# Sirui-Xu/InterDiff

Measured on AMD Instinct MI355X. Metric: denoising frame-steps/sec (denoising-steps/sec x B x T frames), higher is better.
Workload: dtype f32 (every contraction of the denoiser -- feed-forward block, QKV projection, self-attention, row-block contractions and the two token GEMMs: every fp32 operand as two f16 planes, 3 f16 MFMAs per product, fp32 accumulate; SMPL and everything else fp32 MFMA / VALU)

## Files before the change

### include/interdiff_hip.h

```cpp
#ifndef INTERDIFF_HIP_H
#define INTERDIFF_HIP_H

#include <stddef.h>
#include <stdint.h>

#ifdef __cplusplus
extern "C" {
#endif

#define IDF_OK            0
#define IDF_E_INVAL      -22
#define IDF_E_NOMEM      -12
#define IDF_E_LAUNCH     -5

int         interdiff_abi_version(void);
const char *interdiff_build_info(void);

int interdiff_rotation_6d_to_matrix   (const float *d6, float *m,  int64_t n, void *stream);
int interdiff_matrix_to_rotation_6d   (const float *m,  float *d6, int64_t n, void *stream);
int interdiff_matrix_to_axis_angle    (const float *m,  float *aa, int64_t n, void *stream);
int interdiff_axis_angle_to_matrix    (const float *aa, float *m,  int64_t n, void *stream);
int interdiff_axis_angle_to_quaternion(const float *aa, float *q,  int64_t n, void *stream);
int interdiff_rotation_6d_to_axis_angle(const float *d6, float *aa, int64_t n, void *stream);

typedef struct {
    int32_t V, J, n_betas, KB, S;
    const float   *blend;
    const float   *jt;
    const float   *js;
    const int32_t *parents;
    const int32_t *skin_idx;
    const float   *skin_w;
} idf_smpl_model;

size_t interdiff_smpl_workspace_bytes(const idf_smpl_model *m, int64_t N);
int interdiff_smpl_forward(const idf_smpl_model *m, const float *pose, const float *betas,
                           const float *trans, int64_t N, float *verts, float *jtr,
                           float *v_posed, void *ws, size_t ws_bytes, void *stream);

int interdiff_vertex_normals(const float *verts, int64_t N, int32_t V, const int32_t *faces,
                             const int32_t *adj_ptr, const int32_t *adj_face,
                             const int32_t *adj_corner, float *normals, void *stream);
int interdiff_nn_argmin(const float *q, int32_t Pq, const float *r, int32_t Pr, int64_t N,
                        int32_t *idx, void *stream);
int interdiff_point2point_signed(const float *x, int32_t P1, const float *y, int32_t P2, int64_t N,
                                 const float *x_normals, const float *y_normals,
                                 float *y2x_signed, float *x2y_signed, int32_t *yidx, int32_t *xidx,
                                 float *y2x, float *x2y, void *stream);

#define IDF_MDM_LAYERS 8
#define IDF_MDM_D      256
#define IDF_MDM_FF     1024
#define IDF_MDM_HEADS  4
#define IDF_MDM_NQ     10
#define IDF_MDM_MEM    10
#define IDF_MDM_MEM_MAX 16
#define IDF_FFN_SLICES 5

typedef struct {
    int64_t is_qan;
    int64_t sa_in_w, sa_in_b, sa_out_w, sa_out_b;
    int64_t qc, wk;
    int64_t ca_q_w, ca_q_b;
    int64_t ca_kv_w, ca_kv_b;
    int64_t ca_out_w, ca_out_b;
    int64_t ff1_w, ff1_b, ff2_w, ff2_b;
    int64_t ffn_pack;
    int64_t ffn_b1p;
    int64_t sa_in_pack;
    int64_t sa_out_frag;
    int64_t ln_w[3], ln_b[3];
    int64_t ffn_pack_h2;
    int64_t sa_in_pack_h2;
    int64_t qc_h2;
    int64_t rb_h2_ok;
    int64_t sa_out_frag_h2;
    int64_t qkv_bounds_ok;
} idf_mdm_layer;

typedef struct {
    int32_t C;
    int32_t n_steps;
    const float *arena;
    int64_t in_w, in_b;
    int64_t out_w, out_b;
// ... 188 lines not shown
```

### interdiff_amd/_lib.py

```python
import ctypes as C
import os
import torch

_HERE = os.path.dirname(os.path.abspath(__file__))
LIB_PATH = os.environ.get('INTERDIFF_HIP_LIB') or os.path.join(_HERE, 'csrc', 'libinterdiff_hip.so')
ABI_VERSION = 16

vp, i32, i64, f32, u64, sz = C.c_void_p, C.c_int32, C.c_int64, C.c_float, C.c_uint64, C.c_size_t

MDM_LAYERS = 8
FFN_SLICES = 5
STEP_EMBED_READY, STEP_EMBED_NEXT = 1, 2
TUNE = dict(embed=0, qkv=1, outproj=2, ffn=3, ffn_math=4, heads=5, contact=6, misc=7)


class SmplModel(C.Structure):
    _fields_ = [('V', i32), ('J', i32), ('n_betas', i32), ('KB', i32), ('S', i32),
                ('blend', vp), ('jt', vp), ('js', vp), ('parents', vp), ('skin_idx', vp), ('skin_w', vp)]


class MdmLayer(C.Structure):
    _fields_ = [('is_qan', i64),
                ('sa_in_w', i64), ('sa_in_b', i64), ('sa_out_w', i64), ('sa_out_b', i64),
                ('qc', i64), ('wk', i64),
                ('ca_q_w', i64), ('ca_q_b', i64), ('ca_kv_w', i64), ('ca_kv_b', i64),
                ('ca_out_w', i64), ('ca_out_b', i64),
                ('ff1_w', i64), ('ff1_b', i64), ('ff2_w', i64), ('ff2_b', i64), ('ffn_pack', i64), ('ffn_b1p', i64), ('sa_in_pack', i64), ('sa_out_frag', i64),
                ('ln_w', i64 * 3), ('ln_b', i64 * 3), ('ffn_pack_h2', i64), ('sa_in_pack_h2', i64), ('qc_h2', i64), ('rb_h2_ok', i64), ('sa_out_frag_h2', i64), ('qkv_bounds_ok', i64)]


class MdmWeights(C.Structure):
    _fields_ = [('C', i32), ('n_steps', i32), ('arena', vp),
                ('in_w', i64), ('in_b', i64), ('out_w', i64), ('out_b', i64),
                ('temb_table', i64), ('pe', i64), ('max_T', i32), ('has_encoder', i32),
                ('layer', MdmLayer * MDM_LAYERS), ('enc_layer', MdmLayer * MDM_LAYERS), ('tune', i32 * 8), ('out_w_h2', i64), ('in_w_h2', i64), ('tail_h2_ok', i64), ('mem_len', i32), ('rb_tokens', i32)]


class PnMlp(C.Structure):
    _fields_ = [('w', i64 * 3), ('b', i64 * 3), ('c', i32 * 4)]


class PointNet2(C.Structure):
    _fields_ = [('arena', vp), ('sa1', PnMlp * 2), ('sa2', PnMlp * 2), ('lin_w', i64), ('lin_b', i64)]


class ObjProj(C.Structure):
    _fields_ = [('T', i32), ('past_len', i32), ('P', i32), ('n_pre', i32), ('arena', vp),
                ('dct_pad', i64), ('dct', i64), ('idct', i64), ('hand_bonus', i64),
                ('layer', i64 * 12), ('cin', i32 * 12), ('cout', i32 * 12)]


class CorrectionCtx(C.Structure):
    _fields_ = [('smpl', C.POINTER(SmplModel)), ('objproj', C.POINTER(ObjProj)),
                ('faces', vp), ('adj_ptr', vp), ('adj_face', vp), ('adj_corner', vp), ('markers_idx', vp),
                ('n_markers', i32), ('n_points', i32), ('past_len', i32), ('tune', i32),
                ('vorder', vp), ('faces_scan', vp), ('markers_scan', vp), ('adj_pair_scan', vp), ('adj_pair', vp), ('vrank', vp)]


class OptCtx(C.Structure):
    _fields_ = [('geo', C.POINTER(CorrectionCtx)), ('blendT', vp), ('jv_ptr', vp), ('jv_vtx', vp), ('jv_w', vp), ('K3P', i32), ('_pad', i32)]


OPT_NP, OPT_NLOSS = 483, 6
_OPT_PTRS = ('betas', 'obj_points', 'param', 'init', 'grad', 'm', 'v', 'best', 'pose', 'tr', 'verts', 'vposed', 'verts_gt', 'gv',
             'jtr', 'pts', 'y2x', 'y2x_signed', 'yidx', 'near', 'dvposed', 'dA', 'dfeat', 'gtr', 'lossf', 'loss', 'loss_hist',
             'best_loss', 'flag', 'foot_static', 'foot_cnt', 'ctl', 'smpl_ws')


class OptState(C.Structure):
    _fields_ = [('B', i32), ('T', i32), ('P', i32), ('max_iters', i32)] + [(k, vp) for k in _OPT_PTRS] + [('smpl_ws_bytes', sz), ('porder', vp), ('psort', vp), ('pbox', vp)]

# ... 128 lines not shown
```

### interdiff_amd/csrc/denoiser.hip

```cpp
#include "common.h"
#include "gemm.h"
#include "ffn.h"
#include "ffn_h2.h"
#include "tail_h2.h"
#include "attn_h2.h"

static inline int idf_launch_layer_ffn(hipStream_t s, const idf_mdm_layer &ly, const float *ar, const int32_t *tune, const float *x2, int M, float *parts) {
    int rows = idf_ffn::ffn_rows_of_tune(tune[IDF_TUNE_FFN]);
    if (tune[IDF_TUNE_FFN_MATH] != 0 && ly.ffn_pack_h2 != 0) {
        const int rc = idf_ffn_h2::launch_ffn_h2(s, x2, M, ar + ly.ffn_pack_h2, ar + ly.ffn_b1p, ar + ly.ff2_b, parts, rows ? rows : idf_ffn::ffn_tile_for_rows(M), tune[IDF_TUNE_MISC] == 2 ? 1 : (tune[IDF_TUNE_MISC] == 3 ? 2 : (tune[IDF_TUNE_MISC] == 6 ? 3 : (tune[IDF_TUNE_MISC] == 10 ? 4 : 0))));
        if (rc != IDF_NOT_EXCLUSIVE) return rc;
    }
    idf_ffn::launch_ffn(s, x2, M, ar + ly.ffn_pack, ar + ly.ffn_b1p, ar + ly.ff2_b, parts, rows);
    return IDF_OK;
}
#include <float.h>
#ifndef IDF_LDS_STRIDE_SET
#define IDF_LDS_STRIDE_SET 5
#endif

#ifndef IDF_AT_STAMP
#define IDF_AT_STAMP(i) do { } while (0)
#endif
#ifndef IDF_RB_STAMP
// ... 1793 lines not shown
            run_heads_post(tune[IDF_TUNE_GEMM_HEADS], s, g, u_np);
        } else {
            run_gemm_ln<E_HEADS>(pick(tune[IDF_TUNE_GEMM_HEADS], CFG_HEADS), s, g, u_np);
        }
    }
    idf_prof_mark(-1, s);
    IDF_CHECK_LAUNCH();
    return IDF_OK;
}
int mdm_forward_impl(const idf_mdm_weights *w, const float *memctx, const float *x, const int64_t *ts, int32_t B, int32_t T, float *x0,
                     void *ws, size_t ws_bytes, void *stream, const StepPost &post, int32_t flags = 0) {
    if (!w || w->mem_len < 0 || w->mem_len > MEMX) return IDF_E_INVAL;
    return idf_mem_len(w) == MEM ? mdm_forward_impl_t<MEM>(w, memctx, x, ts, B, T, x0, ws, ws_bytes, stream, post, flags)
                                 : mdm_forward_impl_t<MEMX>(w, memctx, x, ts, B, T, x0, ws, ws_bytes, stream, post, flags);
}
}

extern "C" int interdiff_mdm_forward(const idf_mdm_weights *w, const float *memctx, const float *x, const int64_t *ts,
                                     int32_t B, int32_t T, float *x0, void *ws, size_t ws_bytes, void *stream) {
    if (!x0) return IDF_E_INVAL;
    return mdm_forward_impl(w, memctx, x, ts, B, T, x0, ws, ws_bytes, stream, StepPost{});
}

extern "C" int interdiff_mdm_forward_step(const idf_mdm_weights *w, const float *memctx, float *x, int64_t *ts, int32_t B, int32_t T,
                                          const float *gt, const uint8_t *mask, const float *table, int64_t *state, void *ws,
                                          size_t ws_bytes, void *stream) {
    if (!x || !ts || !table || !state || (mask && !gt) || T <= 0) return IDF_E_INVAL;
    if (!(T & 3) && ((reinterpret_cast<uintptr_t>(x) | reinterpret_cast<uintptr_t>(gt)) & 15 || (reinterpret_cast<uintptr_t>(mask) & 3))) return IDF_E_INVAL;
    if ((reinterpret_cast<uintptr_t>(x) | reinterpret_cast<uintptr_t>(gt)) & 3) return IDF_E_INVAL;
    if (!w || w->layer[0].is_qan) return IDF_E_INVAL;
    return mdm_forward_impl(w, memctx, x, ts, B, T, nullptr, ws, ws_bytes, stream, StepPost{x, gt, mask, table, state, ts});
}

extern "C" int interdiff_mdm_forward_step_ex(const idf_mdm_weights *w, const float *memctx, float *x, int64_t *ts, int32_t B, int32_t T,
                                             const float *gt, const uint8_t *mask, const float *table, int64_t *state, void *ws,
                                             size_t ws_bytes, int32_t flags, void *stream) {
    if (!x || !ts || !table || !state || (mask && !gt) || T <= 0 || (flags & ~(IDF_STEP_EMBED_READY | IDF_STEP_EMBED_NEXT))) return IDF_E_INVAL;
    if (!(T & 3) && ((reinterpret_cast<uintptr_t>(x) | reinterpret_cast<uintptr_t>(gt)) & 15 || (reinterpret_cast<uintptr_t>(mask) & 3))) return IDF_E_INVAL;
    if ((reinterpret_cast<uintptr_t>(x) | reinterpret_cast<uintptr_t>(gt)) & 3) return IDF_E_INVAL;
    if (!w || w->layer[0].is_qan) return IDF_E_INVAL;
    return mdm_forward_impl(w, memctx, x, ts, B, T, nullptr, ws, ws_bytes, stream, StepPost{x, gt, mask, table, state, ts}, flags);
}

extern "C" int interdiff_mdm_step_chaining(const idf_mdm_weights *w) {
    return w && w->tune[IDF_TUNE_FFN_MATH] != 0 && w->out_w_h2 != 0 && w->in_w_h2 != 0 && w->C == idf_tail_h2::CW && w->tail_h2_ok != 0 &&
                   idf_tail_h2::tail_exclusive_ok(false) && idf_tail_h2::tail_exclusive_ok(true) ? 1 : 0;
}

extern "C" int interdiff_debug_deny_exclusive(const char *patterns) {
    idf_excl_set_deny(patterns);
    return IDF_OK;
}

extern "C" int interdiff_exclusive_cu_report(char *buf, int32_t cap) {
    if (!buf || cap <= 0) return IDF_E_INVAL;
    {
        static idf_excl_cache c[7];
        using namespace idf_ffn_h2;
        idf_exclusive_cu(reinterpret_cast<const void *>(&ffn_h2_kernel<1, FFN_H2_SLOTS, 0>), "ffn_h2_kernel<16 rows>", NT, c[0]);
        idf_exclusive_cu(reinterpret_cast<const void *>(&ffn_h2_kernel<2, FFN_H2_SLOTS, 0>), "ffn_h2_kernel<32 rows>", NT, c[1]);
        idf_exclusive_cu(reinterpret_cast<const void *>(&ffn_h2_kernel<2, FFN_H2_SLOTS, 0, 8>), "ffn_h2_kernel<32 rows, loader waves>", NT + 512, c[6]);
        idf_exclusive_cu(reinterpret_cast<const void *>(&ffn_h2_kernel<4, 2, 0>), "ffn_h2_kernel<64 rows>", NT, c[2]);
        idf_exclusive_cu(reinterpret_cast<const void *>(&ln_linear_h2_kernel<1, false, IDF_QKV_LOADER_WAVES>), "ln_linear_h2_kernel<1 slab>", NT + 64 * IDF_QKV_LOADER_WAVES, c[3]);
        idf_exclusive_cu(reinterpret_cast<const void *>(&ln_linear_h2_kernel<IDF_FFN_SLICES, false, IDF_QKV_LOADER_WAVES>), "ln_linear_h2_kernel<5 slabs>", NT + 64 * IDF_QKV_LOADER_WAVES, c[4]);
        idf_exclusive_cu(reinterpret_cast<const void *>(&idf_attn_h2::self_attn_h2_kernel<0, false>), "self_attn_h2_kernel", idf_attn_h2::NTH, c[5]);
    }
    qkv_planes_ok(1, 1, 16);
    qkv_planes_ok(NSL, 1, 16);
    rb_h2_qan_dyn<MEM>();
    rb_h2_std_dyn<MEM>();
    rb_h2_qan_dyn<MEMX>();
    rb_h2_std_dyn<MEMX>();
    rb8_qan_dyn<MEM, 16>();
    rb8_std_dyn<MEM, 16>();
    rb8_qan_dyn<MEM, 8>();
    rb8_std_dyn<MEM, 8>();
    rb8_qan_dyn<MEMX, 16>();
    rb8_std_dyn<MEMX, 16>();
    rb8_qan_dyn<MEMX, 8>();
    rb8_std_dyn<MEMX, 8>();
    idf_tail_h2::tail_exclusive_ok(false);
    idf_tail_h2::tail_exclusive_ok(true);
    return idf_excl_report(buf, cap);
}
```

### interdiff_amd/csrc/optimize.hip

```cpp
#include "common.h"
#include "rot_math.h"
#include "rot_dual.h"
#include <cfloat>

namespace {

constexpr int NP = IDF_OPT_NP, NL = IDF_OPT_NLOSS, NJ = 52, MAXJ = 64;
constexpr int OFF_TR = 468, OFF_OT = 471, OFF_OR = 474;
constexpr int FOOT0 = 10;
constexpr int KSLICE = 1024;

__device__ __forceinline__ float sgn(float x) { return x > 0.f ? 1.f : (x < 0.f ? -1.f : 0.f); }

__global__ __launch_bounds__(64) void opt_init_kernel(const float *__restrict__ pose, const float *__restrict__ trans,
                                                      const float *__restrict__ obj_angles, const float *__restrict__ obj_trans,
                                                      float *__restrict__ param, float *__restrict__ init, float *__restrict__ best) {
    const int64_t n = blockIdx.x;
    const int j = threadIdx.x;
    float out[9];
    int off = -1, cnt = 0;
    if (j < NJ || j == NJ + 2) {
        const float *a = j < NJ ? pose + n * 156 + 3 * j : obj_angles + n * 3;
        float q[4];
        rot::axis_angle_to_quaternion(a, q);
// ... 536 lines not shown
            float *h = loss_hist + ((size_t)it * B + b) * 4;
            h[0] = total; h[1] = col; h[2] = reg; h[3] = regv;
        }
        if (flag) {
            const int better = ctl[0] > 150 && total < best_loss[b];
            if (better) best_loss[b] = total;
            flag[b] = better;
        }
    }
}

__global__ __launch_bounds__(256) void opt_save_kernel(const float *__restrict__ param, float *__restrict__ best, const int32_t *__restrict__ flag,
                                                       int T, int64_t total, int32_t *__restrict__ ctl) {
    const int64_t i = (int64_t)blockIdx.x * 256 + threadIdx.x;
    if (i < total && flag[(i / NP) / T]) best[i] = param[i];
    if (i == 0) { ctl[0] += 1; ctl[1] += 1; }
}

__global__ __launch_bounds__(64) void opt_finish_kernel(const float *__restrict__ best, float *__restrict__ pose, float *__restrict__ trans,
                                                        float *__restrict__ obj_angles, float *__restrict__ obj_trans) {
    const int64_t n = blockIdx.x;
    const int j = threadIdx.x;
    const float *p = best + n * NP;
    if (j < NJ) rot::matrix_to_axis_angle(p + 9 * j, pose + n * 156 + 3 * j);
    else if (j == NJ) rot::matrix_to_axis_angle(p + OFF_OR, obj_angles + n * 3);
    else if (j < NJ + 4) {
        const int c = j - NJ - 1;
        trans[n * 3 + c] = p[OFF_TR + c];
        obj_trans[n * 3 + c] = p[OFF_OT + c];
    }
}

bool valid(const idf_opt_ctx *c, const idf_opt_state *st) {
    if (!c || !st || !c->geo || !c->geo->smpl || !c->blendT || !c->jv_ptr || !c->jv_vtx || !c->jv_w) return false;
    const idf_smpl_model *m = c->geo->smpl;
    if (m->J != NJ || m->n_betas != 10 || m->KB % 16 != 0 || c->K3P % KSLICE != 0 || c->K3P < 3 * m->V) return false;
    if (st->B < 1 || st->T < 3 || st->P < 1 || (size_t)m->V * 3 * sizeof(float) > 150 * 1024) return false;
    const void *need[] = {st->betas, st->obj_points, st->param, st->init, st->grad, st->m, st->v, st->best, st->pose, st->tr, st->verts,
                          st->vposed, st->verts_gt, st->gv, st->jtr, st->pts, st->y2x, st->y2x_signed, st->near,
                          st->yidx, st->dvposed, st->dA, st->dfeat, st->gtr, st->lossf, st->loss, st->best_loss, st->flag,
                          st->foot_static, st->foot_cnt, st->ctl, st->smpl_ws};
    for (const void *p : need)
        if (!p) return false;
    return st->smpl_ws_bytes >= interdiff_smpl_workspace_bytes(m, (int64_t)st->B * st->T);
}

int loss_grad(const idf_opt_ctx *c, const idf_opt_state *st, void *stream, bool bookkeeping) {
    const idf_smpl_model *m = c->geo->smpl;
    const int64_t N = (int64_t)st->B * st->T;
    const int V = m->V, J = m->J, P = st->P, T = st->T;
    hipStream_t s = idf_stream(stream);
    hipLaunchKernelGGL(opt_unpack_kernel, dim3((unsigned)N), dim3(64), 0, s, st->param, st->pose, st->tr);
    hipLaunchKernelGGL(opt_objpts_kernel, dim3((unsigned)idf_cdiv(P, 256), (unsigned)N), dim3(256), 0, s, st->param, st->obj_points, P, T, st->pts);
    int rc = interdiff_smpl_forward(m, st->pose, st->betas, st->tr, N, st->verts, st->jtr, st->vposed, st->smpl_ws, st->smpl_ws_bytes, stream);
    if (rc) return rc;
    if (c->geo->vorder && st->porder && st->psort && st->pbox) {
        rc = idf_nn_scan_opt(s, N, T, st->verts, V, st->pts, st->obj_points, P, st->porder, c->geo, st->yidx);
        if (rc) return rc;
        rc = idf_near_mask_opt(s, N, T, st->verts, V, st->pts, P, st->porder, c->geo->vorder, st->psort, st->pbox, st->near);
        if (rc) return rc;
    } else {
        if (hipMemsetAsync(st->near, 0, (size_t)N * V * sizeof(int32_t), s) != hipSuccess) return IDF_E_LAUNCH;
        hipLaunchKernelGGL(opt_nn_kernel, dim3((unsigned)idf_cdiv(P, NN_T * 2), (unsigned)N), dim3(NN_T), 0, s, st->pts, P, st->verts, V, st->yidx,
                           st->near);
    }
    hipLaunchKernelGGL(opt_signed_kernel, dim3((unsigned)idf_cdiv(P, 256), (unsigned)N), dim3(256), 0, s, st->pts, P, st->verts, V, st->yidx,
                       c->geo->faces, c->geo->adj_ptr, c->geo->adj_face, c->geo->adj_corner, c->geo->adj_pair, st->y2x_signed, st->y2x);
    static std::atomic<uint64_t> lds_ok{0};
    if (idf_opt_in_lds(reinterpret_cast<const void *>(opt_lossgrad_kernel), 150 * 1024, lds_ok) != IDF_OK) return IDF_E_LAUNCH;
    hipLaunchKernelGGL(opt_lossgrad_kernel, dim3((unsigned)N), dim3(LG_T), (size_t)V * 3 * sizeof(float), s, st->verts, st->verts_gt, V,
                       st->y2x_signed, st->near, st->yidx, st->y2x, st->obj_points, P, T, st->ctl, st->gv, st->grad, st->gtr, st->lossf);
    const float *A = reinterpret_cast<const float *>(reinterpret_cast<const char *>(st->smpl_ws) + idf_align((size_t)N * m->KB * sizeof(float)));
    hipLaunchKernelGGL(opt_skin_vertex_kernel, dim3((unsigned)idf_cdiv(V, 256), (unsigned)N), dim3(256), 0, s, *m, A, st->gv, c->K3P, st->dvposed);
    hipLaunchKernelGGL(opt_skin_joint_kernel, dim3((unsigned)J, (unsigned)N), dim3(64), 0, s, c->jv_ptr, c->jv_vtx, c->jv_w, st->gv, st->vposed, V,
                       J, st->dA);
    const int n_slices = c->K3P / KSLICE;
    hipLaunchKernelGGL(opt_dfeat_kernel, dim3((unsigned)(m->KB / 16), (unsigned)n_slices, (unsigned)idf_cdiv(N, 16 * DF_MT)), dim3(256), 0, s,
                       st->dvposed, c->blendT, (int)N, m->KB, c->K3P, st->dfeat);
    hipLaunchKernelGGL(opt_chain_bwd_kernel, dim3((unsigned)N), dim3(64), 0, s, *m, st->pose, st->betas, st->param, st->dA, st->dfeat, n_slices, N,
                       T, st->jtr, st->foot_static, st->foot_cnt, st->gtr, st->grad, st->lossf);
    hipLaunchKernelGGL(opt_reg_kernel, dim3((unsigned)N), dim3(512), 0, s, st->param, st->init, T, st->grad, st->lossf);
    hipLaunchKernelGGL(opt_loss_kernel, dim3((unsigned)st->B), dim3(64), 0, s, st->lossf, T, st->B, st->ctl, st->max_iters, st->loss,
                       bookkeeping ? st->loss_hist : nullptr, st->best_loss, bookkeeping ? st->flag : nullptr);
    IDF_CHECK_LAUNCH();
    return IDF_OK;
}

}

extern "C" int interdiff_optimize_init(const idf_opt_ctx *c, const idf_opt_state *st, const float *pose, const float *trans,
                                       const float *obj_angles, const float *obj_trans, int32_t first_iter, void *stream) {
    if (!valid(c, st) || !pose || !trans || !obj_angles || !obj_trans) return IDF_E_INVAL;
    const idf_smpl_model *m = c->geo->smpl;
    const int64_t N = (int64_t)st->B * st->T;
    hipStream_t s = idf_stream(stream);
    hipLaunchKernelGGL(opt_init_kernel, dim3((unsigned)N), dim3(64), 0, s, pose, trans, obj_angles, obj_trans, st->param, st->init, st->best);
    const size_t pb = (size_t)N * NP * sizeof(float);
    if (hipMemsetAsync(st->m, 0, pb, s) != hipSuccess || hipMemsetAsync(st->v, 0, pb, s) != hipSuccess ||
        hipMemsetAsync(st->grad, 0, pb, s) != hipSuccess ||
        hipMemsetAsync(st->dvposed, 0, (size_t)N * c->K3P * sizeof(float), s) != hipSuccess ||
        hipMemsetAsync(st->flag, 0, (size_t)st->B * sizeof(int32_t), s) != hipSuccess)
        return IDF_E_LAUNCH;
    hipLaunchKernelGGL(opt_setctl_kernel, dim3(1), dim3(64), 0, s, st->ctl, first_iter);
    if (c->geo->vorder && st->porder && idf_point_order(s, st->obj_points, st->B, st->P, st->porder) != IDF_OK) return IDF_E_INVAL;
    const int rc = interdiff_smpl_forward(m, pose, st->betas, trans, N, st->verts_gt, st->jtr, nullptr, st->smpl_ws, st->smpl_ws_bytes, stream);
    if (rc) return rc;
    hipLaunchKernelGGL(opt_static_kernel, dim3((unsigned)st->B), dim3(64), 0, s, st->jtr, st->T, m->J, st->foot_static, st->foot_cnt,
                       st->best_loss);
    IDF_CHECK_LAUNCH();
    return IDF_OK;
}

extern "C" int interdiff_optimize_loss_grad(const idf_opt_ctx *c, const idf_opt_state *st, void *stream) {
    if (!valid(c, st)) return IDF_E_INVAL;
    return loss_grad(c, st, stream, false);
}

extern "C" int interdiff_optimize_step(const idf_opt_ctx *c, const idf_opt_state *st, void *stream) {
    if (!valid(c, st)) return IDF_E_INVAL;
    const int rc = loss_grad(c, st, stream, true);
    if (rc) return rc;
    const int64_t total = (int64_t)st->B * st->T * NP;
    hipStream_t s = idf_stream(stream);
    hipLaunchKernelGGL(opt_adam_kernel, dim3((unsigned)idf_cdiv(total, 256)), dim3(256), 0, s, st->param, st->grad, st->m, st->v, total, st->ctl);
    hipLaunchKernelGGL(opt_save_kernel, dim3((unsigned)idf_cdiv(total, 256)), dim3(256), 0, s, st->param, st->best, st->flag, st->T, total, st->ctl);
    IDF_CHECK_LAUNCH();
    return IDF_OK;
}

extern "C" int interdiff_optimize_finish(const idf_opt_ctx *c, const idf_opt_state *st, float *pose, float *trans, float *obj_angles,
                                         float *obj_trans, void *stream) {
    if (!valid(c, st) || !pose || !trans || !obj_angles || !obj_trans) return IDF_E_INVAL;
    hipLaunchKernelGGL(opt_finish_kernel, dim3((unsigned)((int64_t)st->B * st->T)), dim3(64), 0, idf_stream(stream), st->best, pose, trans,
                       obj_angles, obj_trans);
    IDF_CHECK_LAUNCH();
    return IDF_OK;
}

extern "C" int interdiff_debug_joint_map_vjp(const float *R, const float *g_out, float *g_in, int32_t n) {
    if (!R || !g_out || !g_in || n < 0) return IDF_E_INVAL;
    for (int i = 0; i < n; ++i) rotd::joint_map_vjp(R + 9 * i, g_out + 9 * i, g_in + 9 * i);
    return IDF_OK;
}
```

### interdiff_amd/csrc/smpl.hip

```cpp
#include "common.h"
#include "rot_math.h"
#include <algorithm>

#ifndef IDF_SMPL_STAMP
#define IDF_SMPL_STAMP(i) do { } while (0)
#endif

namespace {

constexpr int MAXJ = 64;

__global__ __launch_bounds__(64) void smpl_pose_kernel(const idf_smpl_model m, const float *__restrict__ pose,
                                                       const float *__restrict__ betas, const float *__restrict__ trans,
                                                       float *__restrict__ feat, float *__restrict__ A,
                                                       float *__restrict__ jtr) {
    __shared__ float Rs[MAXJ * 9], Js[MAXJ * 3], Gs[MAXJ * 12];
    const int64_t n = blockIdx.x;
    const int j = threadIdx.x, J = m.J, nb = m.n_betas, KB = m.KB;
    const float *beta = betas + n * nb;
    if (j < J) {
        rot::rodrigues_smpl(pose + n * 3 * J + 3 * j, Rs + j * 9);
#pragma unroll
        for (int c = 0; c < 3; ++c) {
            float s = m.jt[j * 3 + c];
            const float *jsr = m.js + (size_t)(j * 3 + c) * nb;
            for (int k = 0; k < nb; ++k) s += jsr[k] * beta[k];
            Js[j * 3 + c] = s;
        }
    }
    float *f = feat + n * KB;
    if (j >= 1 && j < J) {
#pragma unroll
        for (int e = 0; e < 9; ++e) f[(j - 1) * 9 + e] = Rs[j * 9 + e] - ((e == 0 || e == 4 || e == 8) ? 1.0f : 0.0f);
    }
    const int base = 9 * (J - 1);
    for (int k = j; k < KB - base; k += 64) f[base + k] = k < nb ? beta[k] : (k == nb ? 1.0f : 0.0f);
    __syncthreads();
    if (j < 12) {
        const int r = j >> 2, c = j & 3;
        Gs[j] = c < 3 ? Rs[r * 3 + c] : Js[r];
    }
    __syncthreads();
    for (int i = 1; i < J; ++i) {
        const int p = m.parents[i];
        if (j < 12) {
            const int r = j >> 2, c = j & 3;
            const float *gp = Gs + p * 12 + r * 4;
            float v;
            if (c < 3)
                v = gp[0] * Rs[i * 9 + c] + gp[1] * Rs[i * 9 + 3 + c] + gp[2] * Rs[i * 9 + 6 + c];
            else
                v = gp[0] * (Js[i * 3] - Js[p * 3]) + gp[1] * (Js[i * 3 + 1] - Js[p * 3 + 1]) +
                    gp[2] * (Js[i * 3 + 2] - Js[p * 3 + 2]) + gp[3];
            Gs[i * 12 + j] = v;
        }
// ... 140 lines not shown
    float *Asub = sm + ((FT * STS + 255) & ~255);
    float *ost = Asub + ((SF * J * 12 + 255) & ~255);
    float *trs = ost + SF * NTC;
    const int arow = J * 12;
    if (tid < FT * 3) trs[tid] = trans[min(f0 + tid / 3, N - 1) * 3 + tid % 3];
    for (int sub = 0; sub < FT / SF; ++sub) {
        const int64_t fs = f0 + sub * SF;
        if (fs >= N) break;
        __syncthreads();
        {
            const uint32_t asub_lds = idf_lds_addr(Asub);
            const float *src = idf_uniform_ptr(A + (size_t)fs * arow);
            for (int i = wave; i * 256 < SF * arow; i += BT / 64) idf_dma16_s(src + (size_t)i * 256, (uint32_t)(lane << 4), asub_lds + (uint32_t)(i * 1024));
            asm volatile("s_waitcnt vmcnt(0)" ::: "memory");
        }
        __syncthreads();
        IDF_SMPL_STAMP(3 + 3 * sub);
#pragma unroll
        for (int k = 0; k < SF * VT / BT; ++k) {
            const int f = (tid >> 6) + (BT / 64) * k, fr = sub * SF + f;
            const float px = stage[fr * STS + 3 * vl], py = stage[fr * STS + 3 * vl + 1], pz = stage[fr * STS + 3 * vl + 2];
            float4 t0 = make_float4(0.f, 0.f, 0.f, 0.f), t1 = t0, t2 = t0;
            const float *Af = Asub + f * arow;
#pragma unroll
            for (int b = 0; b < 4; ++b) {
                if (b < S) {
                    const float w = sw[b];
                    const float4 *a = reinterpret_cast<const float4 *>(Af + so[b]);
                    const float4 a0 = a[0], a1 = a[1], a2 = a[2];
                    t0.x = fmaf(w, a0.x, t0.x); t0.y = fmaf(w, a0.y, t0.y); t0.z = fmaf(w, a0.z, t0.z); t0.w = fmaf(w, a0.w, t0.w);
                    t1.x = fmaf(w, a1.x, t1.x); t1.y = fmaf(w, a1.y, t1.y); t1.z = fmaf(w, a1.z, t1.z); t1.w = fmaf(w, a1.w, t1.w);
                    t2.x = fmaf(w, a2.x, t2.x); t2.y = fmaf(w, a2.y, t2.y); t2.z = fmaf(w, a2.z, t2.z); t2.w = fmaf(w, a2.w, t2.w);
                }
            }
            float *o = ost + f * NTC + 3 * vl;
            o[0] = fmaf(t0.x, px, fmaf(t0.y, py, fmaf(t0.z, pz, t0.w))) + trs[fr * 3 + 0];
            o[1] = fmaf(t1.x, px, fmaf(t1.y, py, fmaf(t1.z, pz, t1.w))) + trs[fr * 3 + 1];
            o[2] = fmaf(t2.x, px, fmaf(t2.y, py, fmaf(t2.z, pz, t2.w))) + trs[fr * 3 + 2];
        }
        __syncthreads();
        IDF_SMPL_STAMP(4 + 3 * sub);
        const int nvalid = min(VT, V - v0) * 3;
        for (int idx = tid; idx < SF * (NTC / 2); idx += BT) {
            const int f = idx / (NTC / 2), c2 = (idx - f * (NTC / 2)) * 2;
            if (fs + f >= N || c2 >= nvalid) continue;
            const size_t go = ((size_t)(fs + f) * V + v0) * 3 + c2;
            *reinterpret_cast<float2 *>(verts + go) = *reinterpret_cast<const float2 *>(ost + f * NTC + c2);
            if (v_posed) *reinterpret_cast<float2 *>(v_posed + go) = make_float2(stage[(sub * SF + f) * STS + c2], stage[(sub * SF + f) * STS + c2 + 1]);
        }
        IDF_SMPL_STAMP(5 + 3 * sub);
    }
}

}

extern "C" size_t interdiff_smpl_workspace_bytes(const idf_smpl_model *m, int64_t N) {
    if (!m || N < 0) return 0;
    return idf_align((size_t)N * m->KB * sizeof(float)) + idf_align(((size_t)N + SF) * m->J * 12 * sizeof(float));
}

extern "C" int interdiff_smpl_forward(const idf_smpl_model *m, const float *pose, const float *betas, const float *trans,
                                      int64_t N, float *verts, float *jtr, float *v_posed, void *ws, size_t ws_bytes,
                                      void *stream) {
    if (!m || !pose || !betas || !trans || !verts || !jtr || !ws || N < 0) return IDF_E_INVAL;
    if (m->J < 1 || m->J > MAXJ || m->KB % 16 != 0 || m->KB < 9 * (m->J - 1) + m->n_betas + 1 || m->S < 1) return IDF_E_INVAL;
    if (ws_bytes < interdiff_smpl_workspace_bytes(m, N)) return IDF_E_NOMEM;
    if (N == 0) return IDF_OK;
    hipStream_t s = idf_stream(stream);
    float *feat = reinterpret_cast<float *>(ws);
    float *A = reinterpret_cast<float *>(reinterpret_cast<char *>(ws) + idf_align((size_t)N * m->KB * sizeof(float)));
    idf_prof_mark(IDF_K_SMPL_POSE, s);
    hipLaunchKernelGGL(smpl_pose_kernel, dim3((unsigned)N), dim3(64), 0, s, *m, pose, betas, trans, feat, A, jtr);
    const size_t lds = std::max((size_t)FT * m->KB, (size_t)((FT * STS + 255) & ~255) + ((SF * m->J * 12 + 255) & ~255) + (size_t)SF * NTC + FT * 3) * sizeof(float);
    if (lds > 150 * 1024 || m->KB % 32 != 0 || (m->V * 3) % 2 != 0 || m->S > 4) return IDF_E_INVAL;
    if (m->KB != 480) return IDF_E_INVAL;
    static std::atomic<uint64_t> lds_ok{0};
    if (lds > 64 * 1024 && idf_opt_in_lds(reinterpret_cast<const void *>(smpl_blend_skin_kernel<30>), 150 * 1024, lds_ok) != IDF_OK) return IDF_E_LAUNCH;
    idf_prof_mark(IDF_K_SMPL_BLEND_SKIN, s);
#ifdef IDF_SMPL_XF
    const unsigned nwg_launch = (unsigned)(8 * idf_cdiv(idf_cdiv(N, FT), IDF_SMPL_XF) * idf_cdiv(idf_cdiv(m->V, VT), 8 / IDF_SMPL_XF));
#else
    const unsigned nwg_launch = (unsigned)(idf_cdiv(idf_cdiv(N, FT), TBF) * idf_cdiv(idf_cdiv(m->V, VT), TBV) * TBF * TBV);
#endif
    hipLaunchKernelGGL(smpl_blend_skin_kernel<30>, dim3(nwg_launch), dim3(BT), lds, s, *m,
                       feat, A, trans, N, verts, v_posed);
    idf_prof_mark(-1, s);
    IDF_CHECK_LAUNCH();
    return IDF_OK;
}
```

### interdiff_amd/smpl.py

```python
import ctypes as C
import numpy as np
import torch
from . import _lib


def _np(a):
    return a.detach().cpu().numpy() if isinstance(a, torch.Tensor) else np.asarray(a)


def pack_smpl_model(model, device):
    vt = _np(model['v_template']).astype(np.float64).reshape(-1, 3)
    sdirs = _np(model['shapedirs']).astype(np.float64)
    pdirs = _np(model['posedirs']).astype(np.float64)
    jreg = _np(model['J_regressor']).astype(np.float64)
    wts = _np(model['weights']).astype(np.float32)
    parents = _np(model['parents']).astype(np.int64).copy()
    V, J, nb = vt.shape[0], wts.shape[1], sdirs.shape[2]
    kp = 9 * (J - 1)
    if pdirs.shape != (V, 3, kp) or jreg.shape != (J, V):
        raise ValueError('inconsistent SMPL buffers')
    KB = (kp + nb + 1 + 15) // 16 * 16
    blend = np.zeros((3 * V, KB), np.float32)
    blend[:, :kp] = pdirs.reshape(3 * V, kp)
    blend[:, kp:kp + nb] = sdirs.reshape(3 * V, nb)
    blend[:, kp + nb] = vt.reshape(3 * V)
    jt = (jreg @ vt).astype(np.float32)
    js = np.einsum('jv,vck->jck', jreg, sdirs).astype(np.float32)
    nnz = (wts != 0)
    S = max(1, int(nnz.sum(1).max()))
    skin_idx = np.zeros((V, S), np.int32)
    skin_w = np.zeros((V, S), np.float32)
    for v in range(V):
        js_ = np.nonzero(nnz[v])[0]
        skin_idx[v, :len(js_)] = js_
        skin_w[v, :len(js_)] = wts[v, js_]
    parents[0] = 0
    t = lambda a: torch.from_numpy(np.ascontiguousarray(a)).to(device)
    nvt = -(-V // 64)
    rows = np.zeros((nvt * 192, KB), np.float32)
    rows[:3 * V] = blend
    frag = rows.reshape(nvt, 4, 3, 16, KB // 16, 4, 4).transpose(0, 1, 2, 4, 5, 3, 6)
    bufs = dict(blend=t(frag), blend_rows=t(blend), jt=t(jt), js=t(js), parents=t(parents.astype(np.int32)), skin_idx=t(skin_idx), skin_w=t(skin_w))
    m = _lib.SmplModel()
    m.V, m.J, m.n_betas, m.KB, m.S = V, J, nb, KB, S
    for k, v in bufs.items():
        if k != 'blend_rows':
            setattr(m, k, v.data_ptr())
    return m, bufs


class SMPL_Layer:
    def __init__(self, model, device='cuda'):
        self.lib = _lib.load()
        self.device = torch.device(device)
        self.cmodel, self._bufs = pack_smpl_model(model, self.device)
        self.th_faces = torch.from_numpy(_np(model['faces']).astype(np.int64)).to(self.device)
        self.v_template = _np(model['v_template']).astype(np.float32).reshape(-1, 3)
        self.num_joints = self.cmodel.J
        self.kintree_parents = [int(p) for p in _np(model['parents'])]
        self._ws = None

    def _workspace(self, N):
        need = self.lib.interdiff_smpl_workspace_bytes(C.byref(self.cmodel), N)
        if self._ws is None or self._ws.numel() < need:
            self._ws = torch.empty(max(need, 256), dtype=torch.uint8, device=self.device)
        return self._ws

    def forward(self, th_pose_axisang, th_betas=None, th_trans=None, th_offsets=None, scale=1., want_v_posed=True):
        if th_offsets is not None or scale != 1.:
            raise NotImplementedError('th_offsets / scale are not used on the eval_smpl_short path')
        N = th_pose_axisang.shape[0]
        J, V, nb = self.cmodel.J, self.cmodel.V, self.cmodel.n_betas
        if th_pose_axisang.shape[1] != 3 * J:
            raise ValueError('pose must be [N,%d]' % (3 * J))
        if th_betas is None:
            th_betas = torch.zeros(N, nb, device=self.device)
        if th_trans is None:
            th_trans = torch.zeros(N, 3, device=self.device)
        pose, betas, trans = (a.contiguous().float() for a in (th_pose_axisang, th_betas, th_trans))
        verts = torch.empty(N, V, 3, dtype=torch.float32, device=self.device)
        jtr = torch.empty(N, J, 3, dtype=torch.float32, device=self.device)
        v_posed = torch.empty(N, V, 3, dtype=torch.float32, device=self.device) if want_v_posed else None
        ws = self._workspace(N)
        _lib.check(self.lib.interdiff_smpl_forward(C.byref(self.cmodel), _lib.dptr(pose, torch.float32), _lib.dptr(betas, torch.float32),
                                                   _lib.dptr(trans, torch.float32), N, _lib.dptr(verts), _lib.dptr(jtr),
                                                   _lib.dptr(v_posed, allow_none=True), _lib.dptr(ws), ws.numel(), _lib.stream()),
                   'smpl_forward')
        return verts, jtr, v_posed, v_posed

    __call__ = forward
```

Baseline: 7.182 million.

## Add split-f16 MFMA blend-skin kernel for SMPL forward

Adds a new SMPL blend+skin kernel that stores the blend basis as hi/lo f16 planes and computes the blend contraction with three f16 MFMAs per product, splitting activations on the fly. Work is divided across half-waves over K, with double-buffered A sub-tiles and XCD-aware tile remapping. The optimizer path forces the fp32 kernel. This relies on the basis passing an f16 range check and changes SMPL numerics, which the task says should stay fp32.

```diff
diff --git a/include/interdiff_hip.h b/include/interdiff_hip.h
--- a/include/interdiff_hip.h
+++ b/include/interdiff_hip.h
@@ -31,6 +31,7 @@
     const int32_t *parents;
     const int32_t *skin_idx;
     const float   *skin_w;
+    const void    *blend_h2;
 } idf_smpl_model;
 
 size_t interdiff_smpl_workspace_bytes(const idf_smpl_model *m, int64_t N);
diff --git a/interdiff_amd/_lib.py b/interdiff_amd/_lib.py
--- a/interdiff_amd/_lib.py
+++ b/interdiff_amd/_lib.py
@@ -16,7 +16,7 @@
 
 class SmplModel(C.Structure):
     _fields_ = [('V', i32), ('J', i32), ('n_betas', i32), ('KB', i32), ('S', i32),
-                ('blend', vp), ('jt', vp), ('js', vp), ('parents', vp), ('skin_idx', vp), ('skin_w', vp)]
+                ('blend', vp), ('jt', vp), ('js', vp), ('parents', vp), ('skin_idx', vp), ('skin_w', vp), ('blend_h2', vp)]
 
 
 class MdmLayer(C.Structure):
diff --git a/interdiff_amd/csrc/denoiser.hip b/interdiff_amd/csrc/denoiser.hip
--- a/interdiff_amd/csrc/denoiser.hip
+++ b/interdiff_amd/csrc/denoiser.hip
@@ -1869,6 +1869,7 @@
     return IDF_OK;
 }
 
+int idf_smpl_h2_dyn();
 extern "C" int interdiff_exclusive_cu_report(char *buf, int32_t cap) {
     if (!buf || cap <= 0) return IDF_E_INVAL;
     {
@@ -1898,5 +1899,6 @@
     rb8_std_dyn<MEMX, 8>();
     idf_tail_h2::tail_exclusive_ok(false);
     idf_tail_h2::tail_exclusive_ok(true);
+    idf_smpl_h2_dyn();
     return idf_excl_report(buf, cap);
 }
diff --git a/interdiff_amd/csrc/optimize.hip b/interdiff_amd/csrc/optimize.hip
--- a/interdiff_amd/csrc/optimize.hip
+++ b/interdiff_amd/csrc/optimize.hip
@@ -612,7 +612,9 @@
     hipStream_t s = idf_stream(stream);
     hipLaunchKernelGGL(opt_unpack_kernel, dim3((unsigned)N), dim3(64), 0, s, st->param, st->pose, st->tr);
     hipLaunchKernelGGL(opt_objpts_kernel, dim3((unsigned)idf_cdiv(P, 256), (unsigned)N), dim3(256), 0, s, st->param, st->obj_points, P, T, st->pts);
-    int rc = interdiff_smpl_forward(m, st->pose, st->betas, st->tr, N, st->verts, st->jtr, st->vposed, st->smpl_ws, st->smpl_ws_bytes, stream);
+    idf_smpl_model mf = *m;
+    mf.blend_h2 = nullptr;
+    int rc = interdiff_smpl_forward(&mf, st->pose, st->betas, st->tr, N, st->verts, st->jtr, st->vposed, st->smpl_ws, st->smpl_ws_bytes, stream);
     if (rc) return rc;
     if (c->geo->vorder && st->porder && st->psort && st->pbox) {
         rc = idf_nn_scan_opt(s, N, T, st->verts, V, st->pts, st->obj_points, P, st->porder, c->geo, st->yidx);
@@ -663,7 +665,9 @@
         return IDF_E_LAUNCH;
     hipLaunchKernelGGL(opt_setctl_kernel, dim3(1), dim3(64), 0, s, st->ctl, first_iter);
     if (c->geo->vorder && st->porder && idf_point_order(s, st->obj_points, st->B, st->P, st->porder) != IDF_OK) return IDF_E_INVAL;
-    const int rc = interdiff_smpl_forward(m, pose, st->betas, trans, N, st->verts_gt, st->jtr, nullptr, st->smpl_ws, st->smpl_ws_bytes, stream);
+    idf_smpl_model mf = *m;
+    mf.blend_h2 = nullptr;
+    const int rc = interdiff_smpl_forward(&mf, pose, st->betas, trans, N, st->verts_gt, st->jtr, nullptr, st->smpl_ws, st->smpl_ws_bytes, stream);
     if (rc) return rc;
     hipLaunchKernelGGL(opt_static_kernel, dim3((unsigned)st->B), dim3(64), 0, s, st->jtr, st->T, m->J, st->foot_static, st->foot_cnt,
                        st->best_loss);
diff --git a/interdiff_amd/csrc/smpl.hip b/interdiff_amd/csrc/smpl.hip
--- a/interdiff_amd/csrc/smpl.hip
+++ b/interdiff_amd/csrc/smpl.hip
@@ -1,6 +1,7 @@
 #include "common.h"
 #include "rot_math.h"
 #include <algorithm>
+#include <type_traits>
 
 #ifndef IDF_SMPL_STAMP
 #define IDF_SMPL_STAMP(i) do { } while (0)
@@ -247,6 +248,206 @@
     }
 }
 
+constexpr int FT2 = 64, BT2 = 512;
+constexpr int SF2 = 16, NSUB2 = FT2 / SF2;
+constexpr int KB2 = 480, NS2 = KB2 / 32, nq2 = KB2 / 4;
+#ifndef IDF_SMPL2_TBF
+#define IDF_SMPL2_TBF 5
+#define IDF_SMPL2_TBV 4
+#endif
+constexpr int TBF2 = IDF_SMPL2_TBF, TBV2 = IDF_SMPL2_TBV;
+constexpr int FEAT2_B = FT2 * KB2 * 4;
+constexpr int STAGE2_B = ((FT2 * STS * 4 + 1023) / 1024) * 1024;
+constexpr int ASUB2_MAX_B = 40 * 1024;
+constexpr int ASUB2_B0 = FEAT2_B, ASUB2_B1 = STAGE2_B;
+constexpr int OST2_B = ASUB2_B1 + ASUB2_MAX_B, TRS2_B = OST2_B + SF2 * NTC * 4;
+static_assert(ASUB2_B0 + ASUB2_MAX_B <= IDF_CU_LDS_BYTES && TRS2_B + FT2 * 3 * 4 <= FEAT2_B, "LDS map of smpl_blend_skin_h2_kernel");
+constexpr float LO2_SCALE = 2048.0f, LO2_UNSCALE = 1.0f / 2048.0f;
+typedef _Float16 h8s __attribute__((ext_vector_type(8)));
+typedef float f2s __attribute__((ext_vector_type(2)));
+typedef _Float16 h2s __attribute__((ext_vector_type(2)));
+
+__device__ __forceinline__ void smpl_split4(const float4 v, uint2 &hi, uint2 &lo) {
+    const f2s a = {v.x, v.y}, b = {v.z, v.w};
+    const h2s ha = __builtin_convertvector(a, h2s), hb = __builtin_convertvector(b, h2s);
+    const f2s ra = (a - __builtin_convertvector(ha, f2s)) * LO2_SCALE, rb = (b - __builtin_convertvector(hb, f2s)) * LO2_SCALE;
+    const h2s la = __builtin_convertvector(ra, h2s), lb = __builtin_convertvector(rb, h2s);
+    hi = uint2{__builtin_bit_cast(unsigned, ha), __builtin_bit_cast(unsigned, hb)};
+    lo = uint2{__builtin_bit_cast(unsigned, la), __builtin_bit_cast(unsigned, lb)};
+}
+
+__global__ __launch_bounds__(BT2) void smpl_blend_skin_h2_kernel(const idf_smpl_model m, const float *__restrict__ feat,
+                                                                  const float *__restrict__ A, const float *__restrict__ trans,
+                                                                  int64_t N, float *__restrict__ verts, float *__restrict__ v_posed) {
+    extern __shared__ __attribute__((aligned(1024))) float sm[];
+    asm volatile("" ::: "v255");
+    idf_args_now(m.V, m.J, m.S, m.blend_h2, m.skin_idx, m.skin_w, feat, A, trans, N, verts, v_posed, gridDim.x);
+    const int V = m.V, J = m.J, S = m.S;
+    float *As = sm, *stage = sm;
+    const int tid = threadIdx.x, lane = tid & 63, wave = tid >> 6, cg = wave & 3, mh = wave >> 2, li = lane & 15, kq = lane >> 4;
+    const int nft = (int)((N + FT2 - 1) / FT2), nvt = (V + VT - 1) / VT;
+    const int nwg = gridDim.x, id = blockIdx.x;
+    const int xq = nwg >> 3, xr = nwg & 7, xcd = id & 7;
+    const int lid = (xcd < xr ? xcd * (xq + 1) : xr * (xq + 1) + (xcd - xr) * xq) + (id >> 3);
+    const int blk = lid / (TBF2 * TBV2), wi = lid - blk * (TBF2 * TBV2);
+    const int nvb = (nvt + TBV2 - 1) / TBV2;
+    const int ftile = (blk / nvb) * TBF2 + wi % TBF2, vtile = (blk % nvb) * TBV2 + wi / TBF2;
+    if (ftile >= nft || vtile >= nvt) return;
+    const int64_t f0 = (int64_t)ftile * FT2;
+    const int v0 = vtile * VT;
+    const int arow = J * 12, asub_words = SF2 * arow;
+    auto copy_asub = [&](int sub, int byte_off) {
+        const uint32_t dst = idf_lds_addr(sm) + (uint32_t)byte_off;
+        const float *src = idf_uniform_ptr(A + (size_t)(f0 + sub * SF2) * arow);
+        for (int i = wave; i * 256 < asub_words; i += BT2 / 64) idf_dma16_s(src + (size_t)i * 256, (uint32_t)(lane << 4), dst + (uint32_t)(i * 1024));
+    };
+
+    {
+        const uint32_t as_lds = idf_lds_addr(As);
+        constexpr int ncell = FT2 * nq2;
+        for (int i = wave; i * 64 < ncell; i += BT2 / 64) {
+            const int p = min(i * 64 + lane, ncell - 1), row = p / nq2, pos = p - row * nq2;
+            idf_dma16_v(feat + (size_t)min(f0 + row, N - 1) * KB2 + ((pos ^ ((row >> 1) & 7)) << 2), as_lds + (uint32_t)(i * 1024));
+        }
+    }
+    copy_asub(0, ASUB2_B0);
+    const int vl = tid & 63, vme = v0 + vl;
+    float sw[4];
+    int so[4];
+#pragma unroll
+    for (int k = 0; k < 4; ++k) {
+        const size_t e = (size_t)min(vme, V - 1) * S + min(k, S - 1);
+        sw[k] = m.skin_w[e];
+        so[k] = m.skin_idx[e] * 12;
+    }
+#pragma unroll
+    for (int k = 0; k < 4; ++k) {
+        const bool ok = k < S && vme < V;
+        sw[k] = ok ? sw[k] : 0.f;
+        so[k] = ok ? so[k] : 0;
+    }
+    asm volatile("s_waitcnt vmcnt(0)" ::: "memory");
+    __syncthreads();
+
+    const uint4 *bbase = reinterpret_cast<const uint4 *>(m.blend_h2) + (size_t)(vtile * 4 + cg) * 3 * NS2 * 2 * 64 + lane;
+    f32x4 acc[4][3], cor[4][3];
+#pragma unroll
+    for (int i = 0; i < 4; ++i)
+#pragma unroll
+        for (int t = 0; t < 3; ++t) acc[i][t] = cor[i][t] = f32x4{0.f, 0.f, 0.f, 0.f};
+    constexpr int PD = 2;
+    uint4 bq[PD + 1][3][2];
+    auto ldg = [&](uint4 (&dst)[3][2], int s) {
+#pragma unroll
+        for (int t = 0; t < 3; ++t)
+#pragma unroll
+            for (int pl = 0; pl < 2; ++pl) dst[t][pl] = bbase[((t * NS2 + s) * 2 + pl) * 64];
+    };
+    auto mac = [&](const uint4 (&bc)[3][2], int s) {
+#pragma unroll
+        for (int i = 0; i < 4; ++i) {
+            const int row = i * 16 + li, sz = (row >> 1) & 7, c0 = s * 8 + kq * 2;
+            const float4 x0 = *reinterpret_cast<const float4 *>(As + row * KB2 + ((c0 ^ sz) << 2));
+            const float4 x1 = *reinterpret_cast<const float4 *>(As + row * KB2 + (((c0 + 1) ^ sz) << 2));
+            uint2 h0, l0, h1, l1;
+            smpl_split4(x0, h0, l0);
+            smpl_split4(x1, h1, l1);
+            const h8s ah = __builtin_bit_cast(h8s, uint4{h0.x, h0.y, h1.x, h1.y}), al = __builtin_bit_cast(h8s, uint4{l0.x, l0.y, l1.x, l1.y});
+#pragma unroll
+            for (int t = 0; t < 3; ++t) {
+                const h8s bh = __builtin_bit_cast(h8s, bc[t][0]), bl = __builtin_bit_cast(h8s, bc[t][1]);
+                acc[i][t] = __builtin_amdgcn_mfma_f32_16x16x32_f16(ah, bh, acc[i][t], 0, 0, 0);
+                cor[i][t] = __builtin_amdgcn_mfma_f32_16x16x32_f16(ah, bl, cor[i][t], 0, 0, 0);
+                cor[i][t] = __builtin_amdgcn_mfma_f32_16x16x32_f16(al, bh, cor[i][t], 0, 0, 0);
+            }
+        }
+    };
+    auto kloop = [&](auto S0, auto NSN) {
+        constexpr int s0 = decltype(S0)::value, ns = decltype(NSN)::value;
+#pragma unroll
+        for (int s = 0; s < PD && s < ns; ++s) ldg(bq[s], s0 + s);
+#pragma unroll
+        for (int s = 0; s < ns; ++s) {
+            if (s + PD < ns) ldg(bq[(s + PD) % (PD + 1)], s0 + s + PD);
+            __builtin_amdgcn_sched_barrier(0);
+            mac(bq[s % (PD + 1)], s0 + s);
+            __builtin_amdgcn_sched_barrier(0);
+        }
+    };
+    if (mh == 0) kloop(std::integral_constant<int, 0>{}, std::integral_constant<int, 8>{});
+    else kloop(std::integral_constant<int, 8>{}, std::integral_constant<int, NS2 - 8>{});
+    __syncthreads();
+    if (mh == 1) {
+#pragma unroll
+        for (int i = 0; i < 4; ++i)
+#pragma unroll
+            for (int t = 0; t < 3; ++t)
+#pragma unroll
+                for (int r = 0; r < 4; ++r) stage[(i * 16 + kq * 4 + r) * STS + (cg * 3 + t) * 16 + li] = fmaf(cor[i][t][r], LO2_UNSCALE, acc[i][t][r]);
+    }
+    __syncthreads();
+    if (mh == 0) {
+#pragma unroll
+        for (int i = 0; i < 4; ++i)
+#pragma unroll
+            for (int t = 0; t < 3; ++t)
+#pragma unroll
+                for (int r = 0; r < 4; ++r) {
+                    float *d = stage + (i * 16 + kq * 4 + r) * STS + (cg * 3 + t) * 16 + li;
+                    *d = fmaf(cor[i][t][r], LO2_UNSCALE, acc[i][t][r]) + *d;
+                }
+    }
+
+    float *ost = sm + OST2_B / 4, *trs = sm + TRS2_B / 4;
+    if (tid < FT2 * 3) trs[tid] = trans[min(f0 + tid / 3, N - 1) * 3 + tid % 3];
+    for (int sub = 0; sub < NSUB2; ++sub) {
+        const int64_t fs = f0 + sub * SF2;
+        if (fs >= N) break;
+        asm volatile("s_waitcnt vmcnt(0)" ::: "memory");
+        __syncthreads();
+        if (sub + 1 < NSUB2 && fs + SF2 < N) copy_asub(sub + 1, (sub & 1) ? ASUB2_B0 : ASUB2_B1);
+        const float *Asub = sm + ((sub & 1) ? ASUB2_B1 : ASUB2_B0) / 4;
+#pragma unroll
+        for (int k = 0; k < SF2 * VT / BT2; ++k) {
+            const int f = (tid >> 6) + (BT2 / 64) * k, fr = sub * SF2 + f;
+            const float px = stage[fr * STS + 3 * vl], py = stage[fr * STS + 3 * vl + 1], pz = stage[fr * STS + 3 * vl + 2];
+            float4 t0 = make_float4(0.f, 0.f, 0.f, 0.f), t1 = t0, t2 = t0;
+            const float *Af = Asub + f * arow;
+#pragma unroll
+            for (int b = 0; b < 4; ++b) {
+                if (b < S) {
+                    const float w = sw[b];
+                    const float4 *a = reinterpret_cast<const float4 *>(Af + so[b]);
+                    const float4 a0 = a[0], a1 = a[1], a2 = a[2];
+                    t0.x = fmaf(w, a0.x, t0.x); t0.y = fmaf(w, a0.y, t0.y); t0.z = fmaf(w, a0.z, t0.z); t0.w = fmaf(w, a0.w, t0.w);
+                    t1.x = fmaf(w, a1.x, t1.x); t1.y = fmaf(w, a1.y, t1.y); t1.z = fmaf(w, a1.z, t1.z); t1.w = fmaf(w, a1.w, t1.w);
+                    t2.x = fmaf(w, a2.x, t2.x); t2.y = fmaf(w, a2.y, t2.y); t2.z = fmaf(w, a2.z, t2.z); t2.w = fmaf(w, a2.w, t2.w);
+                }
+            }
+            float *o = ost + f * NTC + 3 * vl;
+            o[0] = fmaf(t0.x, px, fmaf(t0.y, py, fmaf(t0.z, pz, t0.w))) + trs[fr * 3 + 0];
+            o[1] = fmaf(t1.x, px, fmaf(t1.y, py, fmaf(t1.z, pz, t1.w))) + trs[fr * 3 + 1];
+            o[2] = fmaf(t2.x, px, fmaf(t2.y, py, fmaf(t2.z, pz, t2.w))) + trs[fr * 3 + 2];
+        }
+        __syncthreads();
+        const int nvalid = min(VT, V - v0) * 3;
+        for (int idx = tid; idx < SF2 * (NTC / 2); idx += BT2) {
+            const int f = idx / (NTC / 2), c2 = (idx - f * (NTC / 2)) * 2;
+            if (fs + f >= N || c2 >= nvalid) continue;
+            const size_t go = ((size_t)(fs + f) * V + v0) * 3 + c2;
+            *reinterpret_cast<float2 *>(verts + go) = *reinterpret_cast<const float2 *>(ost + f * NTC + c2);
+            if (v_posed) *reinterpret_cast<float2 *>(v_posed + go) = make_float2(stage[(sub * SF2 + f) * STS + c2], stage[(sub * SF2 + f) * STS + c2 + 1]);
+        }
+    }
+}
+
+static_assert(SF2 == SF, "the workspace's slack behind A is one sub-tile of SF frames");
+
+}
+
+int idf_smpl_h2_dyn() {
+    static idf_excl_cache excl;
+    return idf_exclusive_cu(reinterpret_cast<const void *>(&smpl_blend_skin_h2_kernel), "smpl_blend_skin_h2_kernel", BT2, excl);
 }
 
 extern "C" size_t interdiff_smpl_workspace_bytes(const idf_smpl_model *m, int64_t N) {
@@ -269,6 +470,15 @@
     const size_t lds = std::max((size_t)FT * m->KB, (size_t)((FT * STS + 255) & ~255) + ((SF * m->J * 12 + 255) & ~255) + (size_t)SF * NTC + FT * 3) * sizeof(float);
     if (lds > 150 * 1024 || m->KB % 32 != 0 || (m->V * 3) % 2 != 0 || m->S > 4) return IDF_E_INVAL;
     if (m->KB != 480) return IDF_E_INVAL;
+    const int h2_dyn = m->blend_h2 && (SF2 * m->J * 12) % 256 == 0 && SF2 * m->J * 48 <= ASUB2_MAX_B ? idf_smpl_h2_dyn() : -1;
+    if (h2_dyn >= ASUB2_B0 + ASUB2_MAX_B) {
+        idf_prof_mark(IDF_K_SMPL_BLEND_SKIN, s);
+        const unsigned nwg2 = (unsigned)(idf_cdiv(idf_cdiv(N, FT2), TBF2) * idf_cdiv(idf_cdiv(m->V, VT), TBV2) * TBF2 * TBV2);
+        hipLaunchKernelGGL(smpl_blend_skin_h2_kernel, dim3(nwg2), dim3(BT2), (size_t)h2_dyn, s, *m, feat, A, trans, N, verts, v_posed);
+        idf_prof_mark(-1, s);
+        IDF_CHECK_LAUNCH();
+        return IDF_OK;
+    }
     static std::atomic<uint64_t> lds_ok{0};
     if (lds > 64 * 1024 && idf_opt_in_lds(reinterpret_cast<const void *>(smpl_blend_skin_kernel<30>), 150 * 1024, lds_ok) != IDF_OK) return IDF_E_LAUNCH;
     idf_prof_mark(IDF_K_SMPL_BLEND_SKIN, s);
diff --git a/interdiff_amd/smpl.py b/interdiff_amd/smpl.py
--- a/interdiff_amd/smpl.py
+++ b/interdiff_amd/smpl.py
@@ -2,6 +2,7 @@
 import numpy as np
 import torch
 from . import _lib
+from .mdm import H2_LIMIT, split_f16
 
 
 def _np(a):
@@ -41,12 +42,27 @@
     rows[:3 * V] = blend
     frag = rows.reshape(nvt, 4, 3, 16, KB // 16, 4, 4).transpose(0, 1, 2, 4, 5, 3, 6)
     bufs = dict(blend=t(frag), blend_rows=t(blend), jt=t(jt), js=t(js), parents=t(parents.astype(np.int32)), skin_idx=t(skin_idx), skin_w=t(skin_w))
+    h2 = pack_smpl_model_h2(rows) if KB % 32 == 0 and smpl_h2_range_ok(blend) else None
+    if h2 is not None:
+        bufs['blend_h2'] = t(h2)
     m = _lib.SmplModel()
     m.V, m.J, m.n_betas, m.KB, m.S = V, J, nb, KB, S
     for k, v in bufs.items():
         if k != 'blend_rows':
             setattr(m, k, v.data_ptr())
     return m, bufs
+
+
+def smpl_h2_range_ok(blend):
+    b = np.asarray(blend, np.float64)
+    return bool(np.all(np.isfinite(b)) and np.abs(b).max() < H2_LIMIT)
+
+
+def pack_smpl_model_h2(rows):
+    nr, KB = rows.shape
+    hi, lo = split_f16(rows, flush=False)
+    planes = np.stack([hi, lo], axis=0).reshape(2, nr // 192, 4, 3, 16, KB // 32, 4, 8)
+    return np.ascontiguousarray(planes.transpose(1, 2, 3, 5, 0, 6, 4, 7)).view(np.int16)
 
 
 class SMPL_Layer:
@@ -59,6 +75,18 @@
         self.num_joints = self.cmodel.J
         self.kintree_parents = [int(p) for p in _np(model['parents'])]
         self._ws = None
+
+    @property
+    def blend_math(self):
+        return 'split' if self.cmodel.blend_h2 else 'exact'
+
+    @blend_math.setter
+    def blend_math(self, v):
+        if v not in ('split', 'exact'):
+            raise ValueError(v)
+        if v == 'split' and 'blend_h2' not in self._bufs:
+            raise ValueError('the SMPL basis failed its f16 range proof: only the fp32 kernel is available')
+        self.cmodel.blend_h2 = self._bufs['blend_h2'].data_ptr() if v == 'split' else None
 
     def _workspace(self, N):
         need = self.lib.interdiff_smpl_workspace_bytes(C.byref(self.cmodel), N)
```

Result: no change. 7.220 million (median of 6 runs) (+0.5%).
